# auniquesun/PPT

Hardware: AMD Instinct MI355X
Metric: point-clouds/sec fwd+bwd, PointBERT 1024-pt ModelNet40 (higher is better)
Workload: dtype f16; 1 GPU; C2: ModelNet40 1024-pt PointBERT (ULIP_PointBERT head_type=0, frozen backbone + PromptLearner), train-mode BN + DropPath, fwd + CE(ls 0.2) + bwd + AdamW; feed=resident, per_gpu_batch=32, global_batch=32, npoints=1024, classes=40, parallelism=dp1

## Files before the change

### ppt_amd/csrc/mlp_fused3.hip

```cpp
#include "ppt_common.h"
#include "ppt_act.h"
#include <type_traits>

namespace {

constexpr int D = 384, HID = 1536, HC = 256, NJ = HID / HC;
constexpr int RB = 5, R = 16 * RB;
constexpr int HP = 2 * D + 32, UP = 2 * HC + 32;
constexpr int H2_BYTES = R * HP, U_BYTES = R * UP;
constexpr int LDS_BYTES = H2_BYTES + 2 * U_BYTES + (2 * D + HID + D) * 4;
constexpr int K1 = D / 32, K2 = HC / 32;
#ifndef PPT_MLP3_D1
#define PPT_MLP3_D1 4
#endif
#ifndef PPT_MLP3_D2
#define PPT_MLP3_D2 4
#endif
constexpr int D1 = PPT_MLP3_D1, D2 = PPT_MLP3_D2;
static_assert(K1 % D1 == 0 && K2 % D2 == 0, "ring slots must line up from slab to slab");
static_assert(LDS_BYTES <= 160 * 1024, "LDS");
constexpr int W1_BYTES = HID * D * 2, W2_BYTES = D * HID * 2;

__device__ __forceinline__ float gelu_poly3(float x, float hs)
{
    const float xc = __builtin_amdgcn_fmed3f(x, -4.0f, 4.0f);
    const float u = xc * xc;
    float p = fmaf(-3.161567230e-09f, u, 2.434219084e-07f);
    p = fmaf(p, u, -8.201724995e-06f);
    p = fmaf(p, u, 1.613346976e-04f);
    p = fmaf(p, u, -2.096408280e-03f);
    p = fmaf(p, u, 1.932974532e-02f);
    p = fmaf(p, u, -1.323507577e-01f);
    p = fmaf(p, u, 7.976950407e-01f);
    const float e = p * xc;
    const float h = hs * x;
    return fmaf(h, e, h);
}

#ifdef PPT_MLP3_STAMP
#ifndef PPT_MLP3_STAMP_CHUNK
#define PPT_MLP3_STAMP_CHUNK 0
#endif
#define MLP3_STAMP(j, slot) do { if (lane == 0 && chunk == (int)(blockIdx.x + PPT_MLP3_STAMP_CHUNK * gridDim.x)) stamps[((size_t)(blockIdx.x * 8 + w) * 8 + (j)) * 8 + (slot)] = __builtin_amdgcn_s_memtime(); } while (0)
#else
#define MLP3_STAMP(j, slot) do { } while (0)
#endif

template <typename F>
__global__ __launch_bounds__(512, 2) void vit_mlp3_kernel(const ppt_vit_mlp_params p)
{
    extern __shared__ __align__(16) unsigned char smem[];
    unsigned char *h2 = smem, *ub = smem + H2_BYTES;
    float *gam = reinterpret_cast<float *>(smem + H2_BYTES + 2 * U_BYTES), *bet = gam + D, *b1s = bet + D, *b2s = b1s + HID;
    int lane = threadIdx.x & 63;
    const int w = __builtin_amdgcn_readfirstlane(threadIdx.x >> 6);
    int l15 = lane & 15, kg = lane >> 4, lo16 = lane * 16, tid = threadIdx.x;
#define RELANE() do { asm volatile("" : "+v"(lane)); l15 = lane & 15; kg = lane >> 4; lo16 = lane * 16; tid = 64 * w + lane; } while (0)

    const __amdgpu_buffer_rsrc_t r1 = __builtin_amdgcn_make_buffer_rsrc(const_cast<void *>(p.W1), 0, W1_BYTES, 0x00020000);
    const __amdgpu_buffer_rsrc_t r2 = __builtin_amdgcn_make_buffer_rsrc(const_cast<void *>(p.W2), 0, W2_BYTES, 0x00020000);
    constexpr int WAVE_SLAB = 24 * 1024;
    int o1 = 0, o2 = 0;
    auto next1 = [&](uint4 &fa, uint4 &fb) {
        fa = __builtin_bit_cast(uint4, __builtin_amdgcn_raw_buffer_load_b128(r1, lo16, o1, 0));
        fb = __builtin_bit_cast(uint4, __builtin_amdgcn_raw_buffer_load_b128(r1, lo16 + 1024, o1, 0));
        o1 += 2048;
    };
    auto next2 = [&](uint4 (&f)[3]) {
        f[0] = __builtin_bit_cast(uint4, __builtin_amdgcn_raw_buffer_load_b128(r2, lo16, o2, 0));
        f[1] = __builtin_bit_cast(uint4, __builtin_amdgcn_raw_buffer_load_b128(r2, lo16 + 1024, o2, 0));
        f[2] = __builtin_bit_cast(uint4, __builtin_amdgcn_raw_buffer_load_b128(r2, lo16 + 2048, o2, 0));
        o2 += 3072;
    };
#ifdef PPT_MLP3_STAMP
    unsigned long long *stamps = (unsigned long long *)p.residual2;
#endif

    for (int chunk = blockIdx.x; chunk < p.n_chunks; chunk += gridDim.x) {
        MLP3_STAMP(6, 0);
        RELANE();
        const int row0 = chunk * p.rows_per_chunk;
        const int nrow = min(p.rows_per_chunk, p.M - row0);
        lds_barrier();
        MLP3_STAMP(5, 1);
        ppt_f32x4 acc2[RB][3];
        float hrs[RB], rs1[RB];
        uint4 g1[D1][2], g2[D2][3];
        {
            float cst[6];
            const bool first = chunk == (int)blockIdx.x;
            if (first) {
                const int c = tid;
                cst[0] = c < D ? p.ln_w[c] : 0.f; cst[1] = c < D ? p.ln_b[c] : 0.f; cst[2] = (c < D && p.b2) ? p.b2[c] : 0.f;
#pragma unroll
                for (int i = 0; i < 3; ++i) cst[3 + i] = p.b1 ? p.b1[c + 512 * i] : 0.f;
            }
            if (p.proj_a) {
                const bf16_t *A = (const bf16_t *)p.proj_a;
                for (int i = tid; i < R * (D / 8); i += 512) {
                    const int lr = i / (D / 8), c8 = i % (D / 8);
                    uint4 v = make_uint4(0u, 0u, 0u, 0u);
                    if (lr < nrow) v = *reinterpret_cast<const uint4 *>(A + (size_t)(row0 + lr) * D + 8 * c8);
                    *reinterpret_cast<uint4 *>(h2 + lr * HP + 16 * c8) = v;
                }
            }
            float4 xv[RB][3];
#pragma unroll
            for (int rb = 0; rb < RB; ++rb) {
                const int m = row0 + min(16 * rb + l15, nrow - 1);
#pragma unroll
                for (int nb = 0; nb < 3; ++nb) xv[rb][nb] = *reinterpret_cast<const float4 *>(p.x + (size_t)m * D + 48 * w + 16 * nb + 4 * kg);
            }
#pragma unroll
            for (int rb = 0; rb < RB; ++rb) {
                const int m = row0 + min(16 * rb + l15, nrow - 1);
                hrs[rb] = p.row_scale ? 0.5f * p.row_scale[m / p.row_scale_rows] : 0.5f;
                rs1[rb] = (p.proj_a && p.proj_row_scale) ? p.proj_row_scale[m / p.proj_row_scale_rows] : 1.0f;
            }
            if (first) {
                const int c = tid;
                if (c < D) { gam[c] = cst[0]; bet[c] = cst[1]; b2s[c] = cst[2]; }
#pragma unroll
                for (int i = 0; i < 3; ++i) b1s[c + 512 * i] = cst[3 + i];
            }
            MLP3_STAMP(5, 2);
            if (p.proj_a) {
                const __amdgpu_buffer_rsrc_t wrs = __builtin_amdgcn_make_buffer_rsrc(const_cast<void *>(p.proj_W), 0, 8 * 36 * 64 * 16, 0x00020000);
                auto pfrag = [&](int nb, int ks) {
                    return __builtin_bit_cast(uint4, __builtin_amdgcn_raw_buffer_load_b128(wrs, lo16, (w * 36 + nb * 12 + ks) * 1024, 0));
                };
                uint4 wf[4][3];
#pragma unroll
                for (int ks = 0; ks < 4; ++ks)
#pragma unroll
                    for (int nb = 0; nb < 3; ++nb) wf[ks][nb] = pfrag(nb, ks);
                lds_barrier();
                MLP3_STAMP(5, 3);
#pragma unroll
                for (int rb = 0; rb < RB; ++rb)
#pragma unroll
                    for (int nb = 0; nb < 3; ++nb) acc2[rb][nb] = ppt_f32x4{0.f, 0.f, 0.f, 0.f};
                const unsigned char *ha = h2 + l15 * HP + 16 * kg;
                uint4 fp[2][RB];
#pragma unroll
                for (int rb = 0; rb < RB; ++rb) fp[0][rb] = *reinterpret_cast<const uint4 *>(ha + rb * 16 * HP);
#pragma unroll
                for (int ks = 0; ks < K1; ++ks) {
                    if (ks + 1 < K1) {
#pragma unroll
                        for (int rb = 0; rb < RB; ++rb) fp[(ks + 1) & 1][rb] = *reinterpret_cast<const uint4 *>(ha + rb * 16 * HP + 64 * (ks + 1));
                    }
#pragma unroll
                    for (int rb = 0; rb < RB; ++rb)
#pragma unroll
                        for (int nb = 0; nb < 3; ++nb) acc2[rb][nb] = h16<F>::mfma16(wf[ks & 3][nb], fp[ks & 1][rb], acc2[rb][nb]);
                    if (ks + 4 < K1) {
#pragma unroll
                        for (int nb = 0; nb < 3; ++nb) wf[ks & 3][nb] = pfrag(nb, ks + 4);
                    }
                    __builtin_amdgcn_sched_barrier(0);
                }
                MLP3_STAMP(5, 4);
#pragma unroll
                for (int rb = 0; rb < RB; ++rb) {
                    const float r1 = rs1[rb];
#pragma unroll
                    for (int nb = 0; nb < 3; ++nb) {
                        const int n = 48 * w + 16 * nb + 4 * kg;
                        const float4 bv = p.proj_b ? *reinterpret_cast<const float4 *>(p.proj_b + n) : make_float4(0.f, 0.f, 0.f, 0.f);
                        acc2[rb][nb][0] = (acc2[rb][nb][0] + bv.x) * r1 + xv[rb][nb].x; acc2[rb][nb][1] = (acc2[rb][nb][1] + bv.y) * r1 + xv[rb][nb].y;
                        acc2[rb][nb][2] = (acc2[rb][nb][2] + bv.z) * r1 + xv[rb][nb].z; acc2[rb][nb][3] = (acc2[rb][nb][3] + bv.w) * r1 + xv[rb][nb].w;
                    }
                }
            } else {
#pragma unroll
                for (int rb = 0; rb < RB; ++rb)
#pragma unroll
                    for (int nb = 0; nb < 3; ++nb) acc2[rb][nb] = ppt_f32x4{xv[rb][nb].x, xv[rb][nb].y, xv[rb][nb].z, xv[rb][nb].w};
            }
        }
        MLP3_STAMP(5, 5);
        RELANE();
        o1 = o2 = w * WAVE_SLAB;
#pragma unroll
        for (int s = 0; s < D1; ++s) next1(g1[s][0], g1[s][1]);
#pragma unroll
        for (int s = 0; s < D2; ++s) next2(g2[s]);
        {
            float *psum = reinterpret_cast<float *>(ub);
            float *stat = psum + R * 32;
            if (p.proj_a) lds_barrier();
#pragma unroll
            for (int rb = 0; rb < RB; ++rb) {
                float sum = 0.f;
#pragma unroll
                for (int nb = 0; nb < 3; ++nb) sum += (acc2[rb][nb][0] + acc2[rb][nb][1]) + (acc2[rb][nb][2] + acc2[rb][nb][3]);
                psum[(16 * rb + l15) * 32 + 4 * w + kg] = sum;
            }
            lds_barrier();
            if (tid < R) {
                float t = 0.f;
#pragma unroll
                for (int i = 0; i < 32; ++i) t += psum[tid * 32 + i];
                stat[tid] = t * (1.0f / (float)D);
            }
            lds_barrier();
            float mean_r[RB];
#pragma unroll
            for (int rb = 0; rb < RB; ++rb) {
                const int lr = 16 * rb + l15;
                mean_r[rb] = stat[lr];
                float q = 0.f;
#pragma unroll
                for (int nb = 0; nb < 3; ++nb)
#pragma unroll
                    for (int i = 0; i < 4; ++i) { const float d = acc2[rb][nb][i] - mean_r[rb]; q = fmaf(d, d, q); }
                psum[lr * 32 + 4 * w + kg] = q;
            }
            lds_barrier();
            if (tid < R) {
                float t = 0.f;
#pragma unroll
                for (int i = 0; i < 32; ++i) t += psum[tid * 32 + i];
                stat[R + tid] = 1.0f / sqrtf(t * (1.0f / (float)D) + p.ln_eps);
            }
            lds_barrier();
#pragma unroll
            for (int rb = 0; rb < RB; ++rb) {
                const int lr = 16 * rb + l15;
                const float rstd = stat[R + lr];
#pragma unroll
                for (int nb = 0; nb < 3; ++nb) {
                    const int n = 48 * w + 16 * nb + 4 * kg;
                    const float4 g = *reinterpret_cast<const float4 *>(gam + n), b = *reinterpret_cast<const float4 *>(bet + n);
                    uint2 o = make_uint2(0u, 0u);
                    if (lr < nrow)
                        o = make_uint2(h16<F>::pack2((acc2[rb][nb][0] - mean_r[rb]) * rstd * g.x + b.x, (acc2[rb][nb][1] - mean_r[rb]) * rstd * g.y + b.y),
                                       h16<F>::pack2((acc2[rb][nb][2] - mean_r[rb]) * rstd * g.z + b.z, (acc2[rb][nb][3] - mean_r[rb]) * rstd * g.w + b.w));
                    *reinterpret_cast<uint2 *>(h2 + lr * HP + 2 * n) = o;
                }
            }
        }
        MLP3_STAMP(5, 6);
        lds_barrier();
        MLP3_STAMP(6, 1);
        RELANE();

        ppt_f32x4 a1[RB][2];
        auto gemm1 = [&](int jj) {
#pragma unroll
            for (int h = 0; h < 2; ++h) {
                const float4 bv = *reinterpret_cast<const float4 *>(b1s + jj * HC + 32 * w + 16 * h + 4 * kg);
#pragma unroll
                for (int rb = 0; rb < RB; ++rb) a1[rb][h] = ppt_f32x4{bv.x, bv.y, bv.z, bv.w};
            }
            const unsigned char *ha = h2 + l15 * HP + 16 * kg;
            uint4 fa[2][RB];
#pragma unroll
            for (int rb = 0; rb < RB; ++rb) fa[0][rb] = *reinterpret_cast<const uint4 *>(ha + rb * 16 * HP);
#pragma unroll
            for (int ks = 0; ks < K1; ++ks) {
                if (ks + 1 < K1) {
#pragma unroll
                    for (int rb = 0; rb < RB; ++rb) fa[(ks + 1) & 1][rb] = *reinterpret_cast<const uint4 *>(ha + rb * 16 * HP + 64 * (ks + 1));
                }
                const uint4 wa = g1[ks % D1][0], wb = g1[ks % D1][1];
#pragma unroll
                for (int rb = 0; rb < RB; ++rb) {
                    a1[rb][0] = h16<F>::mfma16(wa, fa[ks & 1][rb], a1[rb][0]);
                    a1[rb][1] = h16<F>::mfma16(wb, fa[ks & 1][rb], a1[rb][1]);
                }
                if (ks + D1 == K1) o1 += 7 * WAVE_SLAB;
                next1(g1[ks % D1][0], g1[ks % D1][1]);
                __builtin_amdgcn_sched_barrier(0);
            }
        };
        auto gelu_pair = [&](int jj, int q) {
            const int rb = q >> 1, h = q & 1;
            float v[4];
#pragma unroll
            for (int i = 0; i < 4; ++i) v[i] = gelu_poly3(a1[rb][h][i], hrs[rb]);
            *reinterpret_cast<uint2 *>(ub + (jj & 1) * U_BYTES + (16 * rb + l15) * UP + (32 * w + 16 * h + 4 * kg) * 2) =
                make_uint2(h16<F>::pack2(v[0], v[1]), h16<F>::pack2(v[2], v[3]));
        };
        auto gemm2 = [&](int j, auto with_gelu_c) {
            constexpr bool with_gelu = decltype(with_gelu_c)::value;
            const unsigned char *ua = ub + (j & 1) * U_BYTES + l15 * UP + 16 * kg;
            uint4 fu[2][RB];
#pragma unroll
            for (int rb = 0; rb < RB; ++rb) fu[0][rb] = *reinterpret_cast<const uint4 *>(ua + rb * 16 * UP);
#pragma unroll
            for (int ks = 0; ks < K2; ++ks) {
                if (ks + 1 < K2) {
#pragma unroll
                    for (int rb = 0; rb < RB; ++rb) fu[(ks + 1) & 1][rb] = *reinterpret_cast<const uint4 *>(ua + rb * 16 * UP + 64 * (ks + 1));
                }
#pragma unroll
                for (int rb = 0; rb < RB; ++rb)
#pragma unroll
                    for (int nb = 0; nb < 3; ++nb) acc2[rb][nb] = h16<F>::mfma16(g2[ks % D2][nb], fu[ks & 1][rb], acc2[rb][nb]);
                if (ks + D2 == K2) o2 += 7 * WAVE_SLAB;
                next2(g2[ks % D2]);
                if constexpr (with_gelu) {
                    gelu_pair(j + 1, ks);
                    if (ks < 2 * RB - K2) gelu_pair(j + 1, K2 + ks);
                }
                __builtin_amdgcn_sched_barrier(0);
            }
        };

        gemm1(0);
#pragma unroll
        for (int q = 0; q < 2 * RB; ++q) gelu_pair(0, q);
        lds_barrier();
        MLP3_STAMP(6, 2);
        for (int j = 0; j < NJ - 1; ++j) {
            MLP3_STAMP(j, 0);
            gemm1(j + 1);
            MLP3_STAMP(j, 1);
            gemm2(j, std::true_type{});
            MLP3_STAMP(j, 2);
            lds_barrier();
            MLP3_STAMP(j, 3);
        }
        MLP3_STAMP(NJ - 1, 0);
        RELANE();
        float4 r2v[RB][3];
#ifndef PPT_MLP3_STAMP
        if (p.residual2) {
#pragma unroll
            for (int rb = 0; rb < RB; ++rb) {
                const int m = row0 + min(16 * rb + l15, nrow - 1);
#pragma unroll
                for (int nb = 0; nb < 3; ++nb) r2v[rb][nb] = *reinterpret_cast<const float4 *>(p.residual2 + (size_t)m * D + 48 * w + 16 * nb + 4 * kg);
            }
        } else
#endif
        {
#pragma unroll
            for (int rb = 0; rb < RB; ++rb)
#pragma unroll
                for (int nb = 0; nb < 3; ++nb) r2v[rb][nb] = make_float4(0.f, 0.f, 0.f, 0.f);
        }
        gemm2(NJ - 1, std::false_type{});
        MLP3_STAMP(7, 0);

#pragma unroll
        for (int rb = 0; rb < RB; ++rb) {
            const int lr = 16 * rb + l15;
            if (lr < nrow) {
                const int m = row0 + lr;
#pragma unroll
                for (int nb = 0; nb < 3; ++nb) {
                    const int n = 48 * w + 16 * nb + 4 * kg;
                    const float4 bv = *reinterpret_cast<const float4 *>(b2s + n);
                    const float r = 2.0f * hrs[rb];
                    const float4 o = make_float4(fmaf(bv.x, r, acc2[rb][nb][0]) + r2v[rb][nb].x, fmaf(bv.y, r, acc2[rb][nb][1]) + r2v[rb][nb].y,
                                                 fmaf(bv.z, r, acc2[rb][nb][2]) + r2v[rb][nb].z, fmaf(bv.w, r, acc2[rb][nb][3]) + r2v[rb][nb].w);
                    *reinterpret_cast<float4 *>(p.out + (size_t)m * D + n) = o;
                }
            }
        }
        MLP3_STAMP(7, 1);
    }
}

__global__ __launch_bounds__(256) void vit_mlp3_retile_kernel(const bf16_t *__restrict__ W1, const bf16_t *__restrict__ W2,
                                                              bf16_t *__restrict__ W1t, bf16_t *__restrict__ W2t)
{
    const int i = blockIdx.x * 256 + threadIdx.x;
    if (i >= NJ * 8 * 24 * 64) return;
    const int lane = i & 63, f = (i >> 6) % 24, w = (i / (64 * 24)) & 7, j = i / (64 * 24 * 8);
    const int l15 = lane & 15, kg = lane >> 4;
    {
        const int ks = f >> 1, h = f & 1;
        *reinterpret_cast<uint4 *>(W1t + (size_t)i * 8) =
            *reinterpret_cast<const uint4 *>(W1 + (size_t)(j * HC + 32 * w + 16 * h + l15) * D + 32 * ks + 8 * kg);
    }
    {
        const int ks = f / 3, nb = f % 3;
        *reinterpret_cast<uint4 *>(W2t + (size_t)i * 8) =
            *reinterpret_cast<const uint4 *>(W2 + (size_t)(48 * w + 16 * nb + l15) * HID + j * HC + 32 * ks + 8 * kg);
    }
}

}

extern "C" int ppt_vit_mlp3_retile(const void *W1, const void *W2, void *W1t, void *W2t, void *stream)
{
    if (!W1 || !W2 || !W1t || !W2t || (((uintptr_t)W1 | (uintptr_t)W2 | (uintptr_t)W1t | (uintptr_t)W2t) & 15)) return PPT_EINVAL;
    hipLaunchKernelGGL(vit_mlp3_retile_kernel, dim3((NJ * 8 * 24 * 64 + 255) / 256), dim3(256), 0, ppt_stream(stream), (const bf16_t *)W1,
                       (const bf16_t *)W2, (bf16_t *)W1t, (bf16_t *)W2t);
    PPT_CHECK_LAUNCH();
    return PPT_OK;
}

extern "C" int ppt_vit_mlp3_bf16(const ppt_vit_mlp_params *pp, void *stream)
{
    if (!pp) return PPT_EINVAL;
    ppt_vit_mlp_params p = *pp;
    if (!p.x || !p.out || !p.W1 || !p.W2 || !p.ln_w || !p.ln_b || p.M <= 0) return PPT_EINVAL;
    if (p.D != D || p.hidden != HID) return PPT_EUNSUPPORTED;
    if (p.dtype != PPT_BF16 && p.dtype != PPT_F16 && p.dtype != 0) return PPT_EINVAL;
    if (p.row_scale && p.row_scale_rows <= 0) return PPT_EINVAL;
    if (((uintptr_t)p.x | (uintptr_t)p.out | (uintptr_t)p.W1 | (uintptr_t)p.W2 | (uintptr_t)p.residual2) & 15) return PPT_EINVAL;
    if (p.proj_a) {
        if (!p.proj_W || (p.proj_row_scale && p.proj_row_scale_rows <= 0)) return PPT_EINVAL;
        if (((uintptr_t)p.proj_a | (uintptr_t)p.proj_W | (uintptr_t)p.proj_b) & 15) return PPT_EINVAL;
    }
    PPT_RAISE_LDS_ONCE(LDS_BYTES, (const void *)vit_mlp3_kernel<bf16_t>, (const void *)vit_mlp3_kernel<f16_t>);
    const int cus = ppt_cu_count(ppt_stream(stream));
    int wgs = p.workgroups > 0 ? p.workgroups : cus;
    int rounds = 1;
    while ((int64_t)rounds * wgs * R < p.M) ++rounds;
    if (p.workgroups <= 0 && ppt_get_persistent_occupancy() < 100) wgs = (int)((p.M + (int64_t)rounds * R - 1) / ((int64_t)rounds * R));
    p.n_chunks = rounds * wgs;
    p.rows_per_chunk = (p.M + p.n_chunks - 1) / p.n_chunks;
    p.n_chunks = (p.M + p.rows_per_chunk - 1) / p.rows_per_chunk;
    const int grid = p.n_chunks < wgs ? p.n_chunks : wgs;
    ppt_launch16(p.dtype, [&](auto f) { hipLaunchKernelGGL(vit_mlp3_kernel<decltype(f)>, dim3(grid), dim3(512), LDS_BYTES, ppt_stream(stream), p); });
    PPT_CHECK_LAUNCH();
    return PPT_OK;
}
```

Before: 12000 point-clouds/s.

## Use direct global-to-LDS DMA and batched prologue loads in fused ViT MLP kernel

Reworks the fused LN+MLP kernel prologue. Constant and proj_a tile staging now uses global_load_lds DMA instead of register round-trips. The x, row-scale and proj-bias loads are issued early and drained with an explicit vmcnt wait, and a PROJ template parameter drops the runtime proj_a branches. The aim is to hide prologue global-load latency before the first GEMM. The cost is hand-counted vmcnt values and inline asm that must stay consistent with the issued loads.

New measurement: 12190 point-clouds/s, median of 6. +1.6%, better.

```diff
diff --git a/ppt_amd/csrc/mlp_fused3.hip b/ppt_amd/csrc/mlp_fused3.hip
--- a/ppt_amd/csrc/mlp_fused3.hip
+++ b/ppt_amd/csrc/mlp_fused3.hip
@@ -37,6 +37,12 @@
     return fmaf(h, e, h);
 }
 
+__device__ __forceinline__ void lds_dma4(const void *gsrc, void *lds)
+{
+    const uint32_t m0v = (uint32_t)(uintptr_t)(__attribute__((address_space(3))) void *)lds;
+    asm volatile("s_mov_b32 m0, %1\n\ts_nop 0\n\tglobal_load_lds_dword %0, off" :: "v"(gsrc), "s"(m0v) : "memory", "m0");
+}
+
 #ifdef PPT_MLP3_STAMP
 #ifndef PPT_MLP3_STAMP_CHUNK
 #define PPT_MLP3_STAMP_CHUNK 0
@@ -46,7 +52,7 @@
 #define MLP3_STAMP(j, slot) do { } while (0)
 #endif
 
-template <typename F>
+template <typename F, bool PROJ>
 __global__ __launch_bounds__(512, 2) void vit_mlp3_kernel(const ppt_vit_mlp_params p)
 {
     extern __shared__ __align__(16) unsigned char smem[];
@@ -84,47 +90,54 @@
         lds_barrier();
         MLP3_STAMP(5, 1);
         ppt_f32x4 acc2[RB][3];
-        float hrs[RB], rs1[RB];
+        float hrs[RB];
         uint4 g1[D1][2], g2[D2][3];
+        auto request_hrs = [&]() {
+            typedef const __attribute__((address_space(1))) float *gfloat_p;
+            const float *rs = p.row_scale;
+            asm volatile("" : "+s"(rs));
+            const gfloat_p rsp = (gfloat_p)(rs ? rs : p.ln_w);
+            const int rsr = rs ? p.row_scale_rows : 0x7fffffff;
+#pragma unroll
+            for (int rb = 0; rb < RB; ++rb) hrs[rb] = rsp[(row0 + min(16 * rb + l15, nrow - 1)) / rsr];
+        };
         {
-            float cst[6];
             const bool first = chunk == (int)blockIdx.x;
+            float4 xv[RB][3];
+            float fac1[RB];
+            auto request_x = [&]() {
+#pragma unroll
+                for (int rb = 0; rb < RB; ++rb) {
+                    const int m = row0 + min(16 * rb + l15, nrow - 1);
+#pragma unroll
+                    for (int nb = 0; nb < 3; ++nb) xv[rb][nb] = *reinterpret_cast<const float4 *>(p.x + (size_t)m * D + 48 * w + 16 * nb + 4 * kg);
+                }
+            };
             if (first) {
-                const int c = tid;
-                cst[0] = c < D ? p.ln_w[c] : 0.f; cst[1] = c < D ? p.ln_b[c] : 0.f; cst[2] = (c < D && p.b2) ? p.b2[c] : 0.f;
-#pragma unroll
-                for (int i = 0; i < 3; ++i) cst[3 + i] = p.b1 ? p.b1[c + 512 * i] : 0.f;
-            }
-            if (p.proj_a) {
-                const bf16_t *A = (const bf16_t *)p.proj_a;
-                for (int i = tid; i < R * (D / 8); i += 512) {
-                    const int lr = i / (D / 8), c8 = i % (D / 8);
-                    uint4 v = make_uint4(0u, 0u, 0u, 0u);
-                    if (lr < nrow) v = *reinterpret_cast<const uint4 *>(A + (size_t)(row0 + lr) * D + 8 * c8);
-                    *reinterpret_cast<uint4 *>(h2 + lr * HP + 16 * c8) = v;
-                }
-            }
-            float4 xv[RB][3];
-#pragma unroll
-            for (int rb = 0; rb < RB; ++rb) {
-                const int m = row0 + min(16 * rb + l15, nrow - 1);
-#pragma unroll
-                for (int nb = 0; nb < 3; ++nb) xv[rb][nb] = *reinterpret_cast<const float4 *>(p.x + (size_t)m * D + 48 * w + 16 * nb + 4 * kg);
-            }
-#pragma unroll
-            for (int rb = 0; rb < RB; ++rb) {
-                const int m = row0 + min(16 * rb + l15, nrow - 1);
-                hrs[rb] = p.row_scale ? 0.5f * p.row_scale[m / p.row_scale_rows] : 0.5f;
-                rs1[rb] = (p.proj_a && p.proj_row_scale) ? p.proj_row_scale[m / p.proj_row_scale_rows] : 1.0f;
-            }
-            if (first) {
-                const int c = tid;
-                if (c < D) { gam[c] = cst[0]; bet[c] = cst[1]; b2s[c] = cst[2]; }
-#pragma unroll
-                for (int i = 0; i < 3; ++i) b1s[c + 512 * i] = cst[3 + i];
-            }
-            MLP3_STAMP(5, 2);
-            if (p.proj_a) {
+#pragma unroll 1
+                for (int k = w; k < (3 * D + HID) / 64; k += 8) {
+                    const float *src = k < D / 64 ? p.ln_w + 64 * k : k < 2 * D / 64 ? p.ln_b + (64 * k - D)
+                                     : k < (2 * D + HID) / 64 ? (p.b1 ? p.b1 + (64 * k - 2 * D) : nullptr) : (p.b2 ? p.b2 + (64 * k - 2 * D - HID) : nullptr);
+                    if (src) lds_dma4(src + lane, gam + 64 * k);
+                    else gam[64 * k + lane] = 0.f;
+                }
+            }
+            if constexpr (PROJ) {
+                if (lane < 2 * D / 16) {
+                    int wv = w;
+                    asm volatile("" : "+s"(wv));
+                    const unsigned char *A = (const unsigned char *)p.proj_a + (size_t)(row0 + wv) * (2 * D) + lo16;
+                    unsigned char *img = h2 + wv * HP;
+#pragma unroll 1
+                    for (int lr = wv; lr < R; lr += 8, A += 8 * 2 * D, img += 8 * HP) {
+                        if (lr < nrow) lds_dma16(A, img);
+                        else {
+                            uint32_t z = 0;
+                            asm volatile("" : "+v"(z));
+                            *reinterpret_cast<uint4 *>(img + lo16) = make_uint4(z, z, z, z);
+                        }
+                    }
+                }
                 const __amdgpu_buffer_rsrc_t wrs = __builtin_amdgcn_make_buffer_rsrc(const_cast<void *>(p.proj_W), 0, 8 * 36 * 64 * 16, 0x00020000);
                 auto pfrag = [&](int nb, int ks) {
                     return __builtin_bit_cast(uint4, __builtin_amdgcn_raw_buffer_load_b128(wrs, lo16, (w * 36 + nb * 12 + ks) * 1024, 0));
@@ -134,6 +147,16 @@
                 for (int ks = 0; ks < 4; ++ks)
 #pragma unroll
                     for (int nb = 0; nb < 3; ++nb) wf[ks][nb] = pfrag(nb, ks);
+                __builtin_amdgcn_sched_barrier(0);
+                request_x();
+                __builtin_amdgcn_sched_barrier(0);
+                const float *rsp1 = p.proj_row_scale ? p.proj_row_scale : p.ln_w;
+                const int rsr1 = p.proj_row_scale ? p.proj_row_scale_rows : 0x7fffffff;
+#pragma unroll
+                for (int rb = 0; rb < RB; ++rb) fac1[rb] = rsp1[(row0 + min(16 * rb + l15, nrow - 1)) / rsr1];
+                request_hrs();
+                MLP3_STAMP(5, 2);
+                asm volatile("s_waitcnt vmcnt(%0)" :: "n"(4 * 3 + RB * 3 + 2 * RB) : "memory");
                 lds_barrier();
                 MLP3_STAMP(5, 3);
 #pragma unroll
@@ -141,6 +164,7 @@
 #pragma unroll
                     for (int nb = 0; nb < 3; ++nb) acc2[rb][nb] = ppt_f32x4{0.f, 0.f, 0.f, 0.f};
                 const unsigned char *ha = h2 + l15 * HP + 16 * kg;
+                float4 bp[3];
                 uint4 fp[2][RB];
 #pragma unroll
                 for (int rb = 0; rb < RB; ++rb) fp[0][rb] = *reinterpret_cast<const uint4 *>(ha + rb * 16 * HP);
@@ -158,21 +182,29 @@
 #pragma unroll
                         for (int nb = 0; nb < 3; ++nb) wf[ks & 3][nb] = pfrag(nb, ks + 4);
                     }
+                    if (ks + 4 == K1) {
+                        const float *pb = p.proj_b ? p.proj_b : p.ln_w;
+#pragma unroll
+                        for (int nb = 0; nb < 3; ++nb) bp[nb] = *reinterpret_cast<const float4 *>(pb + 48 * w + 16 * nb + 4 * kg);
+                    }
                     __builtin_amdgcn_sched_barrier(0);
                 }
                 MLP3_STAMP(5, 4);
 #pragma unroll
                 for (int rb = 0; rb < RB; ++rb) {
-                    const float r1 = rs1[rb];
+                    const float r1 = p.proj_row_scale ? fac1[rb] : 1.0f;
 #pragma unroll
                     for (int nb = 0; nb < 3; ++nb) {
-                        const int n = 48 * w + 16 * nb + 4 * kg;
-                        const float4 bv = p.proj_b ? *reinterpret_cast<const float4 *>(p.proj_b + n) : make_float4(0.f, 0.f, 0.f, 0.f);
+                        const float4 bv = p.proj_b ? bp[nb] : make_float4(0.f, 0.f, 0.f, 0.f);
                         acc2[rb][nb][0] = (acc2[rb][nb][0] + bv.x) * r1 + xv[rb][nb].x; acc2[rb][nb][1] = (acc2[rb][nb][1] + bv.y) * r1 + xv[rb][nb].y;
                         acc2[rb][nb][2] = (acc2[rb][nb][2] + bv.z) * r1 + xv[rb][nb].z; acc2[rb][nb][3] = (acc2[rb][nb][3] + bv.w) * r1 + xv[rb][nb].w;
                     }
                 }
             } else {
+                request_x();
+                request_hrs();
+                if (first) asm volatile("s_waitcnt vmcnt(%0)" :: "n"(RB * 3 + RB) : "memory");
+                MLP3_STAMP(5, 2);
 #pragma unroll
                 for (int rb = 0; rb < RB; ++rb)
 #pragma unroll
@@ -181,6 +213,7 @@
         }
         MLP3_STAMP(5, 5);
         RELANE();
+
         o1 = o2 = w * WAVE_SLAB;
 #pragma unroll
         for (int s = 0; s < D1; ++s) next1(g1[s][0], g1[s][1]);
@@ -189,7 +222,7 @@
         {
             float *psum = reinterpret_cast<float *>(ub);
             float *stat = psum + R * 32;
-            if (p.proj_a) lds_barrier();
+            if constexpr (PROJ) lds_barrier();
 #pragma unroll
             for (int rb = 0; rb < RB; ++rb) {
                 float sum = 0.f;
@@ -310,6 +343,8 @@
         };
 
         gemm1(0);
+#pragma unroll
+        for (int rb = 0; rb < RB; ++rb) hrs[rb] = p.row_scale ? 0.5f * hrs[rb] : 0.5f;
 #pragma unroll
         for (int q = 0; q < 2 * RB; ++q) gelu_pair(0, q);
         lds_barrier();
@@ -408,7 +443,8 @@
         if (!p.proj_W || (p.proj_row_scale && p.proj_row_scale_rows <= 0)) return PPT_EINVAL;
         if (((uintptr_t)p.proj_a | (uintptr_t)p.proj_W | (uintptr_t)p.proj_b) & 15) return PPT_EINVAL;
     }
-    PPT_RAISE_LDS_ONCE(LDS_BYTES, (const void *)vit_mlp3_kernel<bf16_t>, (const void *)vit_mlp3_kernel<f16_t>);
+    PPT_RAISE_LDS_ONCE(LDS_BYTES, (const void *)vit_mlp3_kernel<bf16_t, false>, (const void *)vit_mlp3_kernel<f16_t, false>,
+                       (const void *)vit_mlp3_kernel<bf16_t, true>, (const void *)vit_mlp3_kernel<f16_t, true>);
     const int cus = ppt_cu_count(ppt_stream(stream));
     int wgs = p.workgroups > 0 ? p.workgroups : cus;
     int rounds = 1;
@@ -418,7 +454,10 @@
     p.rows_per_chunk = (p.M + p.n_chunks - 1) / p.n_chunks;
     p.n_chunks = (p.M + p.rows_per_chunk - 1) / p.rows_per_chunk;
     const int grid = p.n_chunks < wgs ? p.n_chunks : wgs;
-    ppt_launch16(p.dtype, [&](auto f) { hipLaunchKernelGGL(vit_mlp3_kernel<decltype(f)>, dim3(grid), dim3(512), LDS_BYTES, ppt_stream(stream), p); });
+    ppt_launch16(p.dtype, [&](auto f) {
+        if (p.proj_a) hipLaunchKernelGGL((vit_mlp3_kernel<decltype(f), true>), dim3(grid), dim3(512), LDS_BYTES, ppt_stream(stream), p);
+        else hipLaunchKernelGGL((vit_mlp3_kernel<decltype(f), false>), dim3(grid), dim3(512), LDS_BYTES, ppt_stream(stream), p);
+    });
     PPT_CHECK_LAUNCH();
     return PPT_OK;
 }
```
